# NoemieJaquier/GaBOtorch

Measured on AMD Instinct MI355X. Metric: SPD affine-invariant kernel-matrix build, pairs/sec (N=4096,d=10), higher is better.
Workload: dtype f64

## Files before the change

gabotorch_amd/_lib.py:

```python
import ctypes
import os

_PKG = os.path.dirname(os.path.abspath(__file__))
LIB_PATH = os.environ.get("GABO_HIP_LIB", os.path.join(_PKG, "libgabo_hip.so"))

GABO_OK = 0
GABO_ERR_DIM, GABO_ERR_ARG, GABO_ERR_NOT_SPD, GABO_ERR_LAUNCH = -1, -2, -3, -4
GABO_OUT_GAUSSIAN, GABO_OUT_DISTANCE, GABO_OUT_LAPLACE, GABO_SYMMETRIC = 0, 1, 2, 4
GABO_OUT_ZONAL = 3
GABO_SPD_REG_MAX_DIM = 12
GABO_SPD_BWD_REG_MAX_DIM = 16
GABO_SPD_FWD_REG_MAX_DIM = 20
GABO_SPD_MAX_DIM = 32
GABO_TR_NESTED_MAX_DIM = 24
(GABO_SPD_EXP, GABO_SPD_LOG, GABO_SPD_INNER, GABO_SPD_NORM, GABO_SPD_DIST, GABO_SPD_EGRAD2RGRAD, GABO_SPD_EHESS2RHESS,
 GABO_SPD_LOGM, GABO_SPD_EXPM, GABO_SPD_SQRTM, GABO_SPD_EIGMAX, GABO_SPD_EIGMIN) = range(12)
GABO_ACQ_EXPECTED_IMPROVEMENT, GABO_ACQ_POSTERIOR_MEAN = 0, 1
GABO_GP_MLL_MAX_N = 160
GABO_GP_FACTOR_MAX_N = 96
GABO_GP_MLL_LARGE_MAX_N = 2048
GABO_GRAM_EIG_MAX_N = 1024
GABO_GRAM_EIG_LDS_MAX_N = 192
GABO_GP_POSTERIOR_MAX_M = 1048576
GABO_MVN_SAMPLE_MAX_M = 192
# ... 15 lines not shown

_c = ctypes
_P, _I64, _I, _D, _SZ = _c.c_void_p, _c.c_int64, _c.c_int, _c.c_double, _c.c_size_t

class AcqParams(_c.Structure):
    _fields_ = [("train_factors", _c.c_void_p), ("alpha", _c.c_void_p), ("linv", _c.c_void_p), ("linv_t", _c.c_void_p),
                ("n", _c.c_int64), ("beta", _c.c_double), ("flags", _c.c_int), ("mean", _c.c_double), ("outputscale", _c.c_double),
                ("kxx", _c.c_double), ("best_f", _c.c_double), ("kind", _c.c_int), ("maximize", _c.c_int), ("out_sign", _c.c_double)]


class SweepConfig(_c.Structure):
    _fields_ = [("acq", AcqParams), ("d", _c.c_int), ("min_eig", _c.c_double), ("max_eig", _c.c_double), ("n_constraints", _c.c_int),
                ("constraint_kind", _c.c_int * 8), ("constraint_bound", _c.c_double * 8), ("strict", _c.c_int),
                ("delta_bar", _c.c_double), ("delta0", _c.c_double), ("delta_cons", _c.c_double), ("theta", _c.c_double), ("kappa", _c.c_double),
                ("mininner", _c.c_int), ("maxinner", _c.c_int), ("rho_prime", _c.c_double), ("rho_regularization", _c.c_double),
                ("mingradnorm", _c.c_double), ("maxiter", _c.c_int64)]


class SphereAcqParams(_c.Structure):
    _fields_ = [("train", _c.c_void_p), ("train_t", _c.c_void_p), ("alpha", _c.c_void_p), ("linv", _c.c_void_p), ("linv_t", _c.c_void_p),
                ("n", _c.c_int64), ("dim", _c.c_int), ("beta", _c.c_double), ("flags", _c.c_int), ("mean", _c.c_double),
                ("outputscale", _c.c_double), ("kxx", _c.c_double), ("best_f", _c.c_double), ("kind", _c.c_int), ("maximize", _c.c_int),
                ("out_sign", _c.c_double), ("series", _c.c_void_p), ("series_levels", _c.c_int), ("series_dim", _c.c_int)]


class SphereSweepConfig(_c.Structure):
    _fields_ = [("acq", SphereAcqParams), ("delta_bar", _c.c_double), ("delta0", _c.c_double), ("theta", _c.c_double), ("kappa", _c.c_double),
                ("mininner", _c.c_int), ("maxinner", _c.c_int), ("exact_hessian", _c.c_int), ("rho_prime", _c.c_double),
                ("rho_regularization", _c.c_double), ("mingradnorm", _c.c_double), ("maxiter", _c.c_int64)]


class SphereSweepConstraints(_c.Structure):
    _fields_ = [("n_constraints", _c.c_int), ("n_equalities", _c.c_int), ("kind", _c.c_int * 8), ("index", _c.c_int * 8), ("bound", _c.c_double * 8),
                ("centres", _c.c_void_p), ("n_centres", _c.c_int), ("strict", _c.c_int), ("delta_cons", _c.c_double)]


class ReconSolveOptions(_c.Structure):
    _fields_ = [(k, _c.c_double) for k in ("bound", "rho_init", "thetarho", "tau", "starting_tolgradnorm", "ending_tolgradnorm", "gammas_fact",
                                          "minstepsize", "maxtime")] + [("maxiter", _c.c_int64)] + \
               [(k, _c.c_double) for k in ("cg_minstepsize", "cg_maxtime", "cg_orth_value")] + [("cg_maxiter", _c.c_int64), ("lookahead", _c.c_int64), ("host_threads", _c.c_int64)]


class ReconSolveLog(_c.Structure):
    _fields_ = [(k, _c.c_int64) for k in ("outer_iterations", "inner_iterations", "evaluations", "launches")] + [("stop_reason", _c.c_int)] + \
               [(k, _c.c_double) for k in ("violation", "rho", "gamma", "final_cost", "seconds", "seconds_evaluator")] + [("host_threads", _c.c_int64)]


ReconEvalFn = _c.CFUNCTYPE(_c.c_int, _c.c_void_p, _c.c_int64, *([_c.POINTER(_c.c_double)] * 7))

SIGNATURES = {
    "gabo_version": (_I, []),
    "gabo_spd_ai_workspace_bytes": (_SZ, [_I64, _I64, _I64, _I]),
    "gabo_spd_ai_pairwise": (_I, [_P, _P, _P, _P, _I64, _I64, _I64, _I, _I64, _I64, _D, _I, _P, _SZ, _P, _P]),
    "gabo_spd_ai_backward": (_I, [_P, _P, _P, _P, _I64, _I64, _I64, _I, _I64, _I64, _I64, _I64, _I64, _D, _I, _P, _SZ, _P, _P]),
    "gabo_spd_ai_backward2_workspace_bytes": (_SZ, [_I64, _I64, _I64, _I]),
    "gabo_spd_ai_backward2": (_I, [_P, _P, _P, _P, _P, _P, _P, _I64, _I64, _I64, _I, _I64, _I64, _I64, _I64, _I64, _D, _I, _P, _SZ, _P, _P]),
    "gabo_nested_spd_gram_workspace_bytes": (_SZ, [_I64, _I64, _I64, _I]),
    "gabo_nested_spd_gram": (_I, [_P, _P, _P, _P, _I64, _I64, _I64, _I, _I, _I, _D, _I, _P, _SZ, _P, _P]),
    "gabo_nested_spd_matern_gram": (_I, [_P, _P, _P, _P, _I64, _I64, _I64, _I, _I, _D, _I, _P, _SZ, _P, _P]),
    "gabo_sphere_pairwise": (_I, [_P, _P, _P, _I64, _I64, _I64, _I, _I64, _I64, _D, _I, _I, _P]),
    "gabo_sphere_ktable_doubles": (_I64, []),
    "gabo_sphere_pairwise_uses_ktable": (_I, [_I64, _I64, _I64, _I, _D, _I, _I]),
    "gabo_sphere_ktable_build": (_I, [_D, _P, _P]),
    "gabo_sphere_pairwise_cached": (_I, [_P, _P, _P, _I64, _I64, _I64, _I, _I64, _I64, _D, _I, _I, _P, _P]),
    "gabo_sphere_from_inner": (_I, [_P, _P, _I64, _D, _I, _I, _P]),
    "gabo_sphere_zonal_from_inner": (_I, [_P, _P, _I64, _P, _I, _I, _P]),
    "gabo_sphere_zonal_pairwise": (_I, [_P, _P, _P, _I64, _I64, _I64, _I, _I64, _I64, _P, _I, _I, _I, _I, _P]),
    "gabo_spd_manifold_op": (_I, [_I, _P, _P, _P, _P, _P, _P, _I64, _I, _P, _P]),
    "gabo_spd_project": (_I, [_P, _P, _P, _I64, _I, _I, _P]),
    "gabo_spd_logm_mandel": (_I, [_P, _P, _I64, _I, _P]),
    "gabo_frobenius_pairwise": (_I, [_P, _P, _P, _I64, _I64, _I64, _I, _I64, _I64, _D, _I, _P]),
    "gabo_gp_acquisition": (_I, [_P, _P, _P, _P, _P, _P, _I64, _I64, _D, _D, _D, _D, _I, _I, _D, _P]),
    "gabo_gp_mll": (_I, [_P, _P, _I64, _D, _D, _D, _D, _P, _P]),
    "gabo_gp_mll_gram": (_I, [_P, _P, _I64, _D, _D, _D, _P, _P, _P]),
    "gabo_gp_mll_series": (_I, [_P, _P, _I64, _P, _P, _I, _I, _D, _D, _D, _P, _P]),
    "gabo_gp_factor": (_I, [_P, _P, _I64, _D, _D, _D, _P, _P, _P, _P, _P, _P]),
    "gabo_gp_mll_large_workspace_bytes": (_SZ, [_I64]),
    "gabo_gp_mll_large": (_I, [_P, _P, _I64, _D, _D, _D, _D, _I, _P, _P, _P, _SZ, _P]),
    "gabo_flat_matern_pairwise": (_I, [_P, _P, _P, _I64, _I64, _I64, _I, _I64, _I64, _D, _I, _P]),
    "gabo_flat_matern_backward": (_I, [_P, _P, _P, _P, _I64, _I64, _I64, _I, _I64, _I64, _I64, _I64, _I64, _D, _I, _D, _P]),
    "gabo_flat_matern_from_distance": (_I, [_P, _P, _I64, _D, _I, _I, _P]),
    "gabo_gp_mll_matern": (_I, [_P, _P, _I64, _D, _I, _D, _D, _D, _P, _P]),
    "gabo_spd_ai_logdiag": (_I, [_P, _P, _P, _I64, _I64, _I, _P]),
    "gabo_spd_ai_spectral_features": (_I, [_P, _P, _P, _P, _P, _I64, _I64, _I, _P]),
    "gabo_gram_extreme_eig_workspace_bytes": (_SZ, [_I64, _I64, _I64]),
    "gabo_gram_extreme_eig": (_I, [_P, _I64, _I64, _P, _I64, _P, _P, _SZ, _P]),
    "gabo_gp_posterior_joint_workspace_bytes": (_SZ, [_I64, _I64]),
    "gabo_gp_posterior_joint": (_I, [_P, _P, _P, _P, _I64, _I64, _D, _D, _P, _P, _P, _SZ, _P]),
    "gabo_mvn_sample": (_I, [_P, _P, _I64, _I64, _c.c_uint64, _P, _P, _P, _P, _P]),
    "gabo_mvn_base_samples": (_I, [_P, _I64, _I64, _c.c_uint64, _P]),
    "gabo_gp_condition_workspace_bytes": (_SZ, [_I64, _I64]),
    "gabo_gp_condition": (_I, [_P, _P, _P, _I64, _P, _P, _P, _I64, _D, _D, _D, _P, _P, _P, _P, _P, _P, _SZ, _P, _P]),
    "gabo_spd_acq_max_train": (_I64, [_I]),
    "gabo_spd_acq_prepare_train": (_I, [_P, _P, _I64, _I, _P, _P]),
    "gabo_spd_acq_eval": (_I, [_P, _P, _P, _P, _P, _P, _P, _P, _I64, _I64, _I, _D, _I, _D, _D, _D, _D, _I, _I, _D, _P, _P, _P]),
    "gabo_spd_tcg_workspace_bytes": (_SZ, [_I64, _I, _I]),
    "gabo_spd_tcg_running_offset": (_SZ, [_I64, _I, _I]),
    "gabo_spd_tcg_begin": (_I, [_P, _P, _P, _P, _P, _P, _P, _SZ, _I64, _I, _I, _P, _P]),
    "gabo_spd_tcg_begin_rand": (_I, [_P, _P, _P, _I64, _I, _I, _P]),
    "gabo_spd_tcg_fd_point": (_I, [_P, _P, _I64, _I, _I, _P]),
    "gabo_spd_tcg_step": (_I, [_P, _P, _P, _I64, _I, _I, _I, _D, _D, _D, _I, _P]),
    "gabo_spd_tcg_end": (_I, [_P, _P, _P, _P, _I64, _I, _I, _P]),
    "gabo_spd_sample": (_I, [_P, _I64, _I, _D, _D, _c.c_uint64, _I, _P]),
    "gabo_spd_sample_range": (_I, [_P, _I64, _I64, _I, _D, _D, _c.c_uint64, _I, _P]),
    "gabo_nested_sphere_epilogue": (_I, [_P, _P, _I64, _I, _D, _I, _P]),
    "gabo_nested_sphere_epilogue_backward": (_I, [_P, _P, _P, _I64, _I, _D, _P]),
# ... 95 lines not shown
```

gabotorch_amd/csrc/riemannian_mean.hip:

```cpp
#include "gabo_device.hpp"
#include "spd_prep.hpp"
#include "spd_eigvec.hpp"
#include "../../include/gabo_hip.h"

#define GABO_MEAN_MAX_DIM 10
#define GABO_MEAN_TWO_WAVE_MAX_DIM 8
#define GABO_MEAN_TWO_PASS_MIN_DIM 4
#define GABO_SPHERE_MEAN_MAX_DIM 512

namespace gabo {

struct MeanPlan {
    int64_t chunks, cpb, P;
};

static int device_cu_count() {
    int dev = 0, v = 0;
    if (hipGetDevice(&dev) == hipSuccess && hipDeviceGetAttribute(&v, hipDeviceAttributeMultiprocessorCount, dev) == hipSuccess && v > 0) return v;
    return 256;
}

static MeanPlan mean_plan(int64_t batch, int64_t n, int waves_per_simd) {
    MeanPlan pl;
    pl.chunks = (n + 63) / 64;
    const int64_t slots = (int64_t)4 * device_cu_count() * waves_per_simd;
    int64_t want = slots / batch;
    if (want < 1) want = 1;
    pl.P = pl.chunks < want ? pl.chunks : want;
    pl.cpb = (pl.chunks + pl.P - 1) / pl.P;
    pl.P = (pl.chunks + pl.cpb - 1) / pl.cpb;
    return pl;
}

__device__ __forceinline__ double weight_scale(const double* __restrict__ weights, int64_t b, int64_t n, int lane) {
    if (!weights) return 1.0 / (double)n;
    double a = 0.0;
    for (int64_t j = lane; j < n; j += 64) a += weights[b * n + j];
    return 1.0 / wave_allsum(a);
}

template <int D>
__global__ __launch_bounds__(64, (D > GABO_MEAN_TWO_WAVE_MAX_DIM ? 1 : 2)) void spd_mean_accumulate_kernel(
    const double* __restrict__ Winv, const double* __restrict__ G, const double* __restrict__ weights, const double* __restrict__ scale,
    double* __restrict__ partial, int64_t n, int P, int64_t cpb, int64_t pstride) {
    constexpr int T = tri_size(D);
    __shared__ double acc[T * 64];
    const int lane = threadIdx.x;
    const int64_t b = blockIdx.x / P;
    const int64_t p = blockIdx.x - b * P;
    const double* W = Winv + b * T;
    const double* Gb = G + b * T * n;
    const double sc = scale[b];
    static_for<T>([&](auto ee) { acc[decltype(ee)::value * 64 + lane] = 0.0; });
    const int64_t jbegin = p * cpb * 64;
    const int64_t jend = (jbegin + cpb * 64 < n) ? jbegin + cpb * 64 : n;
    for (int64_t j0 = jbegin; j0 < jend; j0 += 64) {
        const int64_t j = j0 + lane;
        const bool live = j < n;
        const int64_t jc = live ? j : n - 1;
        const double* Gj = Gb + jc;
        double m[T];
        static_for<T>([&](auto ee) { m[decltype(ee)::value] = 0.0; });
        static_for<D>([&](auto cc) {
            constexpr int col = decltype(cc)::value;
            double g[D - col], c[D - col];
            static_for<D - col>([&](auto kk) { g[decltype(kk)::value] = Gj[(int64_t)tri(col + decltype(kk)::value, col) * n]; });
            static_for<D - col>([&](auto rr) {
                constexpr int r = col + decltype(rr)::value;
                double a = W[tri(r, col)] * g[0];
                static_for<r - col>([&](auto kk) {
                    constexpr int k = col + 1 + decltype(kk)::value;
                    a = __builtin_fma(W[tri(r, k)], g[k - col], a);
                });
// ... 300 lines not shown
```

gabotorch_amd/csrc/spd_pairwise.hip:

```cpp
#include "spd_pairwise_body.hpp"


namespace gabo {
int launch_spd_ai_prepared(int d, double* out, int64_t batch, int64_t n1, int64_t n2, bool shared1, bool shared2, double beta, int flags,
                           double* ws, hipStream_t st) {
    const int64_t s1 = shared1 ? 0 : 1, s2 = shared2 ? 0 : 1;
    switch (d) {
        case 2: return launch_spd_ai<2>(nullptr, nullptr, out, nullptr, batch, n1, n2, s1, s2, beta, flags, ws, nullptr, st, true);
        case 3: return launch_spd_ai<3>(nullptr, nullptr, out, nullptr, batch, n1, n2, s1, s2, beta, flags, ws, nullptr, st, true);
        case 4: return launch_spd_ai<4>(nullptr, nullptr, out, nullptr, batch, n1, n2, s1, s2, beta, flags, ws, nullptr, st, true);
    }
    return GABO_ERR_DIM;
}
}

extern "C" {

size_t gabo_spd_ai_workspace_bytes(int64_t batch, int64_t n1, int64_t n2, int d) {
    if (batch < 0 || n1 < 0 || n2 < 0 || d < 1) return 0;
    const size_t packed = (size_t)(batch * (n1 + n2)) * (size_t)gabo::tri_size(d) * sizeof(double);
    const size_t generic = (size_t)(2 * batch * n1) * (size_t)d * (size_t)d * sizeof(double);
    if (d > GABO_SPD_FWD_REG_MAX_DIM) return generic;
    if (d > GABO_SPD_REG_MAX_DIM) return packed > generic ? packed : generic;
    return packed;
}

int gabo_spd_ai_pairwise(const double* x1, const double* x2, double* out, double* dist_out, int64_t batch, int64_t n1, int64_t n2, int d,
                         int64_t x1_batch_stride, int64_t x2_batch_stride, double beta, int flags, void* workspace,
                         size_t workspace_bytes, int* status, gabo_stream_t stream) {
    if (batch < 0 || n1 < 0 || n2 < 0 || x1_batch_stride < 0 || x2_batch_stride < 0) return GABO_ERR_ARG;
    if (d < 2 || d > GABO_SPD_MAX_DIM) return GABO_ERR_DIM;
    if (batch == 0 || n1 == 0 || n2 == 0) return GABO_OK;
    if (!x1 || !x2 || !out || !workspace || !status) return GABO_ERR_ARG;
    if (workspace_bytes < gabo_spd_ai_workspace_bytes(batch, n1, n2, d)) return GABO_ERR_ARG;
    if ((flags & GABO_SYMMETRIC) && (n1 != n2 || batch > 65535)) return GABO_ERR_ARG;
    hipStream_t st = (hipStream_t)stream;
    double* ws = (double*)workspace;
    if (d > GABO_SPD_FWD_REG_MAX_DIM)
        return gabo::launch_spd_ai_generic(x1, x2, out, dist_out, batch, n1, n2, d, x1_batch_stride, x2_batch_stride, beta, flags, ws,
                                           status, st);
#define GABO_CASE(DD) \
    case DD:          \
        return gabo::launch_spd_ai<DD>(x1, x2, out, dist_out, batch, n1, n2, x1_batch_stride, x2_batch_stride, beta, flags, ws, status, st);
    switch (d) {
#ifdef GABO_ONLY_DIM
        GABO_CASE(GABO_ONLY_DIM)
#else
        GABO_CASE(2) GABO_CASE(3) GABO_CASE(4) GABO_CASE(5) GABO_CASE(6) GABO_CASE(7) GABO_CASE(8) GABO_CASE(9) GABO_CASE(10)
        GABO_CASE(11) GABO_CASE(12)
#endif
    }
#undef GABO_CASE
#ifndef GABO_ONLY_DIM
    if (d > GABO_SPD_REG_MAX_DIM)
        return gabo::launch_spd_ai_wide(d, x1, x2, out, dist_out, batch, n1, n2, x1_batch_stride, x2_batch_stride, beta, flags, ws, status, st);
#endif
    return GABO_ERR_DIM;
}

}
```

gabotorch_amd/csrc/spd_pairwise_body.hpp:

```cpp
#pragma once
#include "gabo_device.hpp"
#include "spd_eig.hpp"
#include "spd_prep.hpp"
#include "gabo_mirror.hpp"
#include "spd_generic.hpp"
#include "gabo_log_tab.hpp"
#include "gabo_exp_tab256.hpp"
#include "gabo_acosh2_table.hpp"
#include "../../include/gabo_hip.h"

#ifndef GABO_PAIR_WAVES
#define GABO_PAIR_WAVES 2
#else
#define GABO_PAIR_WAVES_FORCED 1
#endif

namespace gabo {

typedef const double __attribute__((address_space(1)))* spd_gcol_ptr;

struct SpdGcolBuffer {
    __amdgpu_buffer_rsrc_t rsrc;
    int voff;
    int stride_bytes;
    __device__ __forceinline__ double operator[](int k) const {
        return __builtin_bit_cast(double, __builtin_amdgcn_raw_buffer_load_b64(rsrc, voff, k * stride_bytes, 0));
    }
};
struct SpdGcolPointer {
    spd_gcol_ptr p;
    int64_t stride;
    __device__ __forceinline__ double operator[](int k) const { return p[(int64_t)k * stride]; }
};

template <int D, int WLIM>
struct SpdWGroups {
    int n = 0;
    int col[tri_size(D)] = {}, r0[tri_size(D)] = {}, r1[tri_size(D)] = {};
    constexpr SpdWGroups() {
        static_assert(WLIM >= D, "a row of the first column must fit a group");
        for (int c = D - 1; c >= 0; --c) {
            for (int r = c; r < D;) {
                int sum = 0;
                col[n] = c, r0[n] = r;
                while (r < D && sum + (r - c + 1) <= WLIM) sum += r - c + 1, ++r;
                r1[n++] = r;
            }
        }
    }
};
#ifndef GABO_PAIR_WLIM
#define GABO_PAIR_WLIM 16
#endif
template <int D, int AHEAD, class GCOL>
__device__ __forceinline__ void ai_congruence_staged(const double* __restrict__ W, const GCOL& Gj, double (&m)[tri_size(D)]) {
    constexpr SpdWGroups<D, (GABO_PAIR_WLIM < D ? D : GABO_PAIR_WLIM)> kG{};
    double gq[D][D];
    double wq[2][D][D];
    double c[D];
    auto issue_g = [&](auto ss) {
        constexpr int col = D - 1 - decltype(ss)::value;
// ... 93 lines not shown

struct Spd2Col {
    double g00, g10, g11, lg;
};
__device__ __forceinline__ double ai_sumsq2(const double* __restrict__ W, const Spd2Col& g, double lw, const LogTabRegs& lr,
                                            const double* __restrict__ ltab, double tiny) {
    const double c00 = W[0] * g.g00, c11 = W[2] * g.g11;
    const double c10 = __builtin_fma(W[1], g.g00, W[2] * g.g10);
    const double m00 = c00 * c00, m10d = (c10 + c10) * c00, m11 = __builtin_fma(c10, c10, c11 * c11);
    const double tr = m00 + m11, df = m00 - m11;
    const double root = sqrt_nz(__builtin_fma(df, df, __builtin_fma(m10d, m10d, tiny)));
    const double l1 = log_tab(0.5 * (tr + root), lr, ltab);
    const double l2 = __builtin_fma(2.0, lw + g.lg, -l1);
    return __builtin_fma(l1, l1, l2 * l2);
}

__device__ __forceinline__ double finish(double dist, double beta, int mode) {
    if (mode == GABO_OUT_DISTANCE) return dist;
    if (mode == GABO_OUT_LAPLACE) return exp(-(dist * beta));
    return exp(-((dist * dist) * beta));
}

#ifndef GABO_PAIR_TWO_WAVE_MAX_DIM
#define GABO_PAIR_TWO_WAVE_MAX_DIM 14
#endif
#ifndef GABO_QL_EPS2_GAUSS
#define GABO_QL_EPS2_GAUSS 1e-14
#endif
constexpr bool spd_pair_gauss_only_instantiated(int d) { return d > 2 && d != 12; }
#ifndef GABO_PAIR_ORIENT
constexpr int spd_pair_gauss_only_orientation(int d) { return d == 14 ? kQlOrientCol0 : kQlOrientLast; }
#else
constexpr int spd_pair_gauss_only_orientation(int d) { return GABO_PAIR_ORIENT; }
#endif
#ifndef GABO_PAIR_SWEEPCTL
constexpr int spd_pair_gauss_only_sweepctl(int d) { return d == 20 ? kQlCtlPlain : (kQlCtlDenormalZero | kQlCtlHwSqrt | kQlCtlStageThreshold); }
#else
constexpr int spd_pair_gauss_only_sweepctl(int d) { return GABO_PAIR_SWEEPCTL; }
#endif
#ifndef GABO_PAIR_WAVES_FORCED
constexpr int spd_pair_gauss_only_waves(int d) { return d > GABO_PAIR_TWO_WAVE_MAX_DIM ? 1 : (d == 10 ? 3 : GABO_PAIR_WAVES); }
#else
constexpr int spd_pair_gauss_only_waves(int d) { return d > GABO_PAIR_TWO_WAVE_MAX_DIM ? 1 : GABO_PAIR_WAVES; }
#endif
#ifndef GABO_PAIR_AHEAD
constexpr int spd_pair_gauss_only_ahead(int d) { return d == 10 && spd_pair_gauss_only_waves(d) == 3 ? 2 : 0; }
#else
constexpr int spd_pair_gauss_only_ahead(int d) { return d == 10 ? GABO_PAIR_AHEAD : 0; }
#endif
template <int D, bool GAUSS_ONLY, bool BUFFER_ONLY>
__global__ __launch_bounds__(256, (GAUSS_ONLY ? spd_pair_gauss_only_waves(D) : (D > GABO_PAIR_TWO_WAVE_MAX_DIM ? 1 : GABO_PAIR_WAVES))) void spd_ai_pairwise_kernel(const double* __restrict__ Winv, const double* __restrict__ G,
                                                              double* __restrict__ out, double* __restrict__ dist_out_arg,
                                                              int64_t n1, int64_t n2,
                                                              int64_t w_batch_stride, int64_t g_batch_stride, int rows,
                                                              int col_blocks, int row_chunks, int64_t sym_tiles, double beta, int flags) {
    constexpr int T = tri_size(D);
    static_assert(GAUSS_ONLY == BUFFER_ONLY && (spd_pair_gauss_only_instantiated(D) || !GAUSS_ONLY), "instantiations that launch_spd_ai selects");
    const int mode = GAUSS_ONLY ? GABO_OUT_GAUSSIAN : (flags & GABO_OUT_MASK);
    double* const dist_out = GAUSS_ONLY ? nullptr : dist_out_arg;
    constexpr bool kTabExp = D <= 4;
    __shared__ double tab[kTabExp ? 64 : 1];
    __shared__ __attribute__((aligned(16))) double ltab[512];
    for (int k = threadIdx.x; k < 512; k += blockDim.x) ltab[k] = kLogTab[k];
    double ec[6], ec3 = 0.0;
    if constexpr (kTabExp) {
        if (threadIdx.x < 64) tab[threadIdx.x] = kExp2Tab[threadIdx.x];
    }
    __syncthreads();
    if constexpr (kTabExp) {
        static_for<6>([&](auto k) { ec[decltype(k)::value] = kExpTabC[decltype(k)::value]; });
        ec3 = ec[3];
        asm volatile("" : "+v"(ec3));
    }
    int64_t cg, rc, b;
    if (flags & GABO_SYMMETRIC) {
        const int64_t per_batch = sym_tiles;
        b = blockIdx.x / per_batch;
        int64_t t = blockIdx.x - b * per_batch;
        cg = 0;
        for (;;) {
            int64_t cnt = ((cg + 1) * (int64_t)blockDim.x + rows - 1) / rows;
            if (cnt > row_chunks) cnt = row_chunks;
            if (t < cnt) break;
            t -= cnt;
            ++cg;
        }
        rc = t;
    } else {
        const int64_t bid = blockIdx.x;
        cg = bid % col_blocks;
        rc = (bid / col_blocks) % row_chunks;
        b = bid / ((int64_t)col_blocks * row_chunks);
    }
    const int64_t j0 = cg * blockDim.x;
    const int64_t j = j0 + threadIdx.x;
    const int64_t jc = j < n2 ? j : n2 - 1;
    const int64_t i0 = rc * rows;
    const int64_t i1 = (i0 + rows < n1) ? i0 + rows : n1;
    if ((flags & GABO_SYMMETRIC) && j0 + (int64_t)(threadIdx.x | 63) < i0) return;
    const double* Gj = G + b * g_batch_stride + jc;
    double* ob = out + b * n1 * n2;
    const int64_t jw = j0 + (threadIdx.x & ~63);
    const bool use_buffer = BUFFER_ONLY || (D > 2 && (int64_t)T * n2 * 8 < (1ll << 31));
    SpdGcolBuffer gbuf;
    {
        const double* gw = G + b * g_batch_stride + (jw < n2 ? jw : n2 - 1);
        uint64_t a = (uint64_t)gw;
        a = ((uint64_t)(uint32_t)__builtin_amdgcn_readfirstlane((int)(a >> 32)) << 32) | (uint32_t)__builtin_amdgcn_readfirstlane((int)a);
        gbuf.rsrc = __builtin_amdgcn_make_buffer_rsrc((void*)a, 0, 0x7fffffff, 0x00020000);
        gbuf.voff = (int)((jc - (jw < n2 ? jw : n2 - 1)) * 8);
        gbuf.stride_bytes = (int)(n2 * 8);
    }
    Spd2Col col2;
    double lw_lane = 0.0, tiny = 1e-290;
    LogTabRegs lr2;
    if constexpr (D == 2) {
        lr2 = LogTabRegs::load();
        asm volatile("" : "+s"(tiny));
        col2.g00 = Gj[0];
        col2.g10 = Gj[n2];
        col2.g11 = Gj[2 * n2];
        col2.lg = log_tab(col2.g00 * col2.g11, lr2, ltab);
        int64_t ir = i0 + (threadIdx.x & 63);
        ir = ir < n1 ? ir : n1 - 1;
        const double* Wr = Winv + b * w_batch_stride + ir * T;
        lw_lane = log_tab(Wr[0] * Wr[2], lr2, ltab);
    }
    double eps2 = (mode == GABO_OUT_GAUSSIAN && !dist_out) ? GABO_QL_EPS2_GAUSS : 0.0;
    asm volatile("" : "+s"(eps2));
    if constexpr (GAUSS_ONLY && BUFFER_ONLY) {
        const int nrows = __builtin_amdgcn_readfirstlane((int)(i1 - i0));
        const int64_t jrel = j - i0;
        const int rmax = j >= n2 ? -1 : ((flags & GABO_SYMMETRIC) ? (jrel < 0 ? -1 : (jrel > rows - 1 ? rows - 1 : (int)jrel)) : rows - 1);
        const double* W = Winv + b * w_batch_stride + i0 * T;
        char* orow = reinterpret_cast<char*>(ob + i0 * n2 + j);
        for (int r = 0; r < nrows; ++r, W += T) {
            SpdGcolBuffer gb = gbuf;
            asm volatile("" : "+v"(gb.voff));
            asm volatile("" : "+s"(gb.stride_bytes));
            const double s = ai_sumsq<D, spd_pair_gauss_only_orientation(D), spd_pair_gauss_only_sweepctl(D), spd_pair_gauss_only_ahead(D)>(W, gb, ltab, eps2);
            double val;
            if constexpr (kTabExp) {
                val = exp_neg_tab(-((s + 1e-15) * beta), ec, ec3, tab);
                val = s != s ? s : val;
            } else {
                val = exp(-((s + 1e-15) * beta));
            }
            if (r <= rmax) *reinterpret_cast<double*>(orow) = val;
            orow += (unsigned)gb.stride_bytes;
        }
// ... 124 lines not shown
    const double q00 = g00 * sg, q10 = g10 * sg, q11 = g11 * sg;
    double* orow = out + b * n1 * n2 + i0 * n2 + j;
    const int nrows = __builtin_amdgcn_readfirstlane((int)(i1 - i0));
    const int64_t jrel = j - i0;
    const int rmax = j >= n2 ? -1 : (SYM ? (jrel < 0 ? -1 : (jrel > GABO_GAUSS2_MAX_ROWS - 1 ? GABO_GAUSS2_MAX_ROWS - 1 : (int)jrel)) : GABO_GAUSS2_MAX_ROWS - 1);
    typedef double g2_v2d __attribute__((ext_vector_type(2)));
    if (!SYM && j >= n2) return;
    for (int r = 0; r < nrows; ++r, orow += n2) {
        const g2_v2d wa = *reinterpret_cast<const g2_v2d*>(wrow + 4 * r);
        const g2_v2d wb = *reinterpret_cast<const g2_v2d*>(wrow + 4 * r + 2);
        const double w0 = wa[0], w1 = wa[1], w2 = wb[0], arow = wb[1];
        const double hh = __builtin_fma(w0, q00, -(w2 * q11));
        const double cc = __builtin_fma(w1, q00, w2 * q10);
        const double tau = __builtin_fma(cc, cc, __builtin_fma(hh, hh, 1.0));
        const unsigned hi = (unsigned)__double2hiint(tau);
        static_assert(kAcosh2MBits == 4 && kAcosh2Slots == 256, "row index = 8 bits");
        const unsigned off = __umul24((hi >> 16) & 0xffu, (unsigned)(kAcosh2Stride * sizeof(double)));
        const double t = tau - __hiloint2double((int)(hi & ~((1u << (20 - kAcosh2MBits)) - 1u)), 0);
        const g2_v2d* row = reinterpret_cast<const g2_v2d*>(reinterpret_cast<const char*>(atab) + off);
        static_assert(kAcosh2Deg == 7, "four coefficient pairs");
        const g2_v2d c67 = row[3], c45 = row[2], c23 = row[1], c01 = row[0];
        double ya = __builtin_fma(c67[1], t, c67[0]);
        ya = __builtin_fma(ya, t, c45[1]);
        ya = __builtin_fma(ya, t, c45[0]);
        ya = __builtin_fma(ya, t, c23[1]);
        ya = __builtin_fma(ya, t, c23[0]);
        ya = __builtin_fma(ya, t, c01[1]);
        ya = __builtin_fma(ya, t, c01[0]);
        if (__builtin_expect(__any(!(tau < ec[5])), 0)) {
            if (!(tau < ec[5])) {
                const double dl = log(tau + __builtin_sqrt(__builtin_fma(tau, tau, -1.0)));
                ya = -(sscale * sscale) * __builtin_fma(dl, dl, 0.5e-15);
            }
        }
        const double sp = arow + bcol;
        const double y = __builtin_fma(-sp, sp, ya);
        const double km = y + ec[4];
        const double kk = km - ec[4];
        const double rr = y - kk;
        double p = __builtin_fma(rr, c4v, ec[2]);
        p = __builtin_fma(p, rr, ec[1]);
        p = __builtin_fma(p, rr, ec[0]);
        p = p * rr;
        const int ki = __double2loint(km);
        const double e = etab[ki & 255];
        const double val = __builtin_ldexp(__builtin_fma(e, p, e), ki >> 8);
        if (!SYM || r <= rmax) {
            if constexpr (NT) __builtin_nontemporal_store(val, orow);
            else *orow = val;
        }
    }
}

template <int D>
static int launch_spd_ai(const double* x1, const double* x2, double* out, double* dist_out, int64_t batch, int64_t n1, int64_t n2,
                         int64_t s1, int64_t s2, double beta, int flags, double* ws, int* status, hipStream_t st, bool prepared = false) {
    constexpr int T = tri_size(D);
    const int64_t b1 = (s1 == 0) ? 1 : batch;
    const int64_t b2 = (s2 == 0) ? 1 : batch;
    double* W = ws;
    double* G = ws + b1 * n1 * T;
    if (!prepared) launch_spd_prep<D>(x1, x2, W, G, b1, b2, n1, n2, s1, s2, status, st, 1);
#ifndef GABO_PAIR_THREADS
#define GABO_PAIR_THREADS (D >= 7 ? 64 : 256)
#endif
    int threads = n2 >= 256 ? GABO_PAIR_THREADS : (n2 > 128 ? 192 : (n2 > 64 ? 128 : 64));
    int64_t col_blocks = (n2 + threads - 1) / threads;
#ifndef GABO_PAIR_ROWS_D2
#define GABO_PAIR_ROWS_D2 16
#endif
#ifndef GABO_PAIR_ROWS
#define GABO_PAIR_ROWS (D >= 9 ? 8 : 16)
#endif
#ifndef GABO_PAIR_ROWS_GAUSS2
#define GABO_PAIR_ROWS_GAUSS2 64
#endif
    const bool gauss2 = D == 2 && (flags & GABO_OUT_MASK) == GABO_OUT_GAUSSIAN && !dist_out && beta >= 0.0;
    int rows = D == 2 ? (gauss2 ? GABO_PAIR_ROWS_GAUSS2 : GABO_PAIR_ROWS_D2) : GABO_PAIR_ROWS;
    while (rows > 1 && col_blocks * ((n1 + rows - 1) / rows) * batch < (rows > 16 ? 1024 : 4096)) rows >>= 1;
    int64_t row_chunks = (n1 + rows - 1) / rows;
    int64_t sym_tiles = 0;
    if (flags & GABO_SYMMETRIC) {
        for (int64_t cg = 0; cg < col_blocks; ++cg) {
            int64_t cnt = ((cg + 1) * threads + rows - 1) / rows;
            sym_tiles += cnt < row_chunks ? cnt : row_chunks;
        }
    }
    int64_t nblocks = ((flags & GABO_SYMMETRIC) ? sym_tiles : col_blocks * row_chunks) * batch;
    if (nblocks > 0x7fffffffLL) return GABO_ERR_ARG;
    bool special2 = false;
    if constexpr (D == 2) special2 = gauss2 && rows <= GABO_GAUSS2_MAX_ROWS;
    if (special2) {
        const bool streaming = batch * n1 * n2 * 8 > (32ll << 20) && !(flags & GABO_SYMMETRIC);
#define GABO_GAUSS2_LAUNCH(...)                                                                                                     \
        hipLaunchKernelGGL((spd_ai_gauss2_kernel<__VA_ARGS__>), dim3((unsigned)nblocks), dim3(threads), 0, st, W, G, out, n1, n2,           \
                           (s1 == 0) ? (int64_t)0 : n1 * T, (s2 == 0) ? (int64_t)0 : n2 * T, rows, (int)col_blocks, (int)row_chunks,       \
                           sym_tiles, beta, flags)
        if (flags & GABO_SYMMETRIC) GABO_GAUSS2_LAUNCH(false, true);
        else if (streaming) GABO_GAUSS2_LAUNCH(true, false);
        else GABO_GAUSS2_LAUNCH(false, false);
#undef GABO_GAUSS2_LAUNCH
    } else {
#define GABO_PAIR_LAUNCH(...)                                                                                                             \
        hipLaunchKernelGGL((spd_ai_pairwise_kernel<D, __VA_ARGS__>), dim3((unsigned)nblocks), dim3(threads), 0, st, W, G, out, dist_out, n1, n2, \
                           (s1 == 0) ? (int64_t)0 : n1 * T, (s2 == 0) ? (int64_t)0 : n2 * T, rows, (int)col_blocks, (int)row_chunks,       \
                           sym_tiles, beta, flags)
        bool gauss_only = false;
        if constexpr (spd_pair_gauss_only_instantiated(D)) {
            gauss_only = (flags & GABO_OUT_MASK) == GABO_OUT_GAUSSIAN && !dist_out && (int64_t)T * n2 * 8 < (1ll << 31);
            if (gauss_only) GABO_PAIR_LAUNCH(true, true);
        }
        if (!gauss_only) GABO_PAIR_LAUNCH(false, false);
#undef GABO_PAIR_LAUNCH
    }
    if (flags & GABO_SYMMETRIC) {
        int tiles = (int)((n1 + 31) / 32);
        hipLaunchKernelGGL((mirror_upper_kernel<0>), dim3((unsigned)((int64_t)tiles * (tiles + 1) / 2), (unsigned)batch), dim3(256), 0, st,
                           out, n1, tiles);
        if (dist_out)
            hipLaunchKernelGGL((mirror_upper_kernel<0>), dim3((unsigned)((int64_t)tiles * (tiles + 1) / 2), (unsigned)batch), dim3(256), 0,
                               st, dist_out, n1, tiles);
    }
    return hipGetLastError() == hipSuccess ? GABO_OK : GABO_ERR_LAUNCH;
}

}

namespace gabo {
int launch_spd_ai_prepared(int d, double* out, int64_t batch, int64_t n1, int64_t n2, bool shared1, bool shared2, double beta, int flags,
                           double* ws, hipStream_t st);
int launch_spd_ai_wide2(int d, const double* x1, const double* x2, double* out, double* dist_out, int64_t batch, int64_t n1, int64_t n2,
                        int64_t s1, int64_t s2, double beta, int flags, double* ws, int* status, hipStream_t st);
int launch_spd_ai_wide3(int d, const double* x1, const double* x2, double* out, double* dist_out, int64_t batch, int64_t n1, int64_t n2,
                        int64_t s1, int64_t s2, double beta, int flags, double* ws, int* status, hipStream_t st);
int launch_spd_ai_wide(int d, const double* x1, const double* x2, double* out, double* dist_out, int64_t batch, int64_t n1, int64_t n2,
                       int64_t s1, int64_t s2, double beta, int flags, double* ws, int* status, hipStream_t st);
}
```

include/gabo_hip.h:

```cpp
#ifndef GABO_HIP_H
#define GABO_HIP_H

#include <stddef.h>
#include <stdint.h>

#ifdef __cplusplus
extern "C" {
#endif

typedef void* gabo_stream_t;

#define GABO_OK 0
#define GABO_ERR_DIM (-1)
#define GABO_ERR_ARG (-2)
#define GABO_ERR_NOT_SPD (-3)
#define GABO_ERR_LAUNCH (-4)

#define GABO_OUT_GAUSSIAN 0
#define GABO_OUT_DISTANCE 1
#define GABO_OUT_LAPLACE 2
#define GABO_OUT_ZONAL 3
#define GABO_OUT_MASK 3
#define GABO_SYMMETRIC 4
#define GABO_METRIC_AFFINE_INVARIANT 0
#define GABO_METRIC_LOG_EUCLIDEAN 8
#define GABO_METRIC_FROBENIUS 16
#define GABO_METRIC_MASK 24

#define GABO_SPD_REG_MAX_DIM 12
#define GABO_SPD_BWD_REG_MAX_DIM 16
#define GABO_SPD_FWD_REG_MAX_DIM 20
#define GABO_SPD_MAX_DIM 32

int gabo_version(void);

size_t gabo_spd_ai_workspace_bytes(int64_t batch, int64_t n1, int64_t n2, int d);
int gabo_spd_ai_pairwise(const double* x1, const double* x2, double* out, double* dist_out, int64_t batch, int64_t n1,
                         int64_t n2, int d, int64_t x1_batch_stride, int64_t x2_batch_stride, double beta, int flags,
                         void* workspace, size_t workspace_bytes, int* status, gabo_stream_t stream);

int gabo_spd_ai_backward(const double* x1, const double* x2, const double* grad_out, double* grad_x1, int64_t batch, int64_t n1,
                         int64_t n2, int d, int64_t x1_batch_stride, int64_t x2_batch_stride, int64_t go_batch_stride,
                         int64_t go_row_stride, int64_t go_col_stride, double beta, int flags, void* workspace,
                         size_t workspace_bytes, int* status, gabo_stream_t stream);

size_t gabo_spd_ai_backward2_workspace_bytes(int64_t batch, int64_t n1, int64_t n2, int d);
int gabo_spd_ai_backward2(const double* x1, const double* x2, const double* grad_out, const double* u, double* hv_x1, double* d_grad_out,
                          double* mixed_x2, int64_t batch, int64_t n1, int64_t n2, int d, int64_t x1_batch_stride, int64_t x2_batch_stride,
                          int64_t go_batch_stride, int64_t go_row_stride, int64_t go_col_stride, double beta, int flags, void* workspace,
                          size_t workspace_bytes, int* status, gabo_stream_t stream);

int gabo_sphere_pairwise(const double* x1, const double* x2, double* out, int64_t batch, int64_t n1, int64_t n2,
                         int dim, int64_t x1_batch_stride, int64_t x2_batch_stride, double beta, int flags, int diag,
                         gabo_stream_t stream);
int64_t gabo_sphere_ktable_doubles(void);
int gabo_sphere_pairwise_uses_ktable(int64_t batch, int64_t n1, int64_t n2, int dim, double beta, int flags, int diag);
int gabo_sphere_ktable_build(double beta, double* table, gabo_stream_t stream);
int gabo_sphere_pairwise_cached(const double* x1, const double* x2, double* out, int64_t batch, int64_t n1, int64_t n2,
                                int dim, int64_t x1_batch_stride, int64_t x2_batch_stride, double beta, int flags, int diag,
                                const double* ktable, gabo_stream_t stream);

int gabo_sphere_from_inner(const double* inner, double* out, int64_t n, double beta, int flags, int order, gabo_stream_t stream);

int gabo_sphere_zonal_from_inner(const double* inner, double* out, int64_t n, const double* coeff_host, int n_coeff, int series_dim,
                                 gabo_stream_t stream);
int gabo_sphere_zonal_pairwise(const double* x1, const double* x2, double* out, int64_t batch, int64_t n1, int64_t n2, int dim,
                               int64_t x1_batch_stride, int64_t x2_batch_stride, const double* coeff_host, int n_coeff, int series_dim,
                               int flags, int diag, gabo_stream_t stream);

int gabo_mandel_to_matrix(const double* vec, double* mat, int64_t n, int d, gabo_stream_t stream);
int gabo_matrix_to_mandel(const double* mat, double* vec, int64_t n, int d, gabo_stream_t stream);

#define GABO_SPD_EXP 0
#define GABO_SPD_LOG 1
#define GABO_SPD_INNER 2
#define GABO_SPD_NORM 3
#define GABO_SPD_DIST 4
#define GABO_SPD_EGRAD2RGRAD 5
#define GABO_SPD_EHESS2RHESS 6
#define GABO_SPD_LOGM 7
#define GABO_SPD_EXPM 8
#define GABO_SPD_SQRTM 9
#define GABO_SPD_EIGMAX 10
#define GABO_SPD_EIGMIN 11
int gabo_spd_manifold_op(int op, const double* a, const double* b, const double* c, const double* e, double* out, double* out2,
                         int64_t n, int d, int* status, gabo_stream_t stream);

int gabo_spd_project(const double* x_mandel, const double* w, double* y_mandel, int64_t n, int D, int dl, gabo_stream_t stream);

int gabo_spd_logm_mandel(const double* x_mandel, double* y_mandel, int64_t n, int d, gabo_stream_t stream);

int gabo_frobenius_pairwise(const double* x1, const double* x2, double* out, int64_t batch, int64_t n1, int64_t n2, int d,
// ... 375 lines not shown
```

Baseline: 7.976 billion.

## Shrink row-chunk sizes near the end of the grid to balance the final wave

Replaces the uniform rows-per-block split of the SPD affine-invariant pairwise kernel with a multi-phase row schedule. The bulk of the rows keeps the default chunk size, and the tail of the last batch is split into progressively smaller power-of-two chunks, sized from an estimate of how many wave slots the device has. The aim is to shorten the partially filled last wave of blocks. The CU count query is now cached per device, and an API entry exposes the computed schedule. In exchange, block-index decoding in the kernel becomes more complex, and the small tail chunks reuse x1 rows less.

```diff
diff --git a/gabotorch_amd/_lib.py b/gabotorch_amd/_lib.py
--- a/gabotorch_amd/_lib.py
+++ b/gabotorch_amd/_lib.py
@@ -91,6 +91,7 @@
     "gabo_version": (_I, []),
     "gabo_spd_ai_workspace_bytes": (_SZ, [_I64, _I64, _I64, _I]),
     "gabo_spd_ai_pairwise": (_I, [_P, _P, _P, _P, _I64, _I64, _I64, _I, _I64, _I64, _D, _I, _P, _SZ, _P, _P]),
+    "gabo_spd_ai_row_schedule": (_I, [_I64, _I64, _I64, _I, _I, _I64, _P, _I]),
     "gabo_spd_ai_backward": (_I, [_P, _P, _P, _P, _I64, _I64, _I64, _I, _I64, _I64, _I64, _I64, _I64, _D, _I, _P, _SZ, _P, _P]),
     "gabo_spd_ai_backward2_workspace_bytes": (_SZ, [_I64, _I64, _I64, _I]),
     "gabo_spd_ai_backward2": (_I, [_P, _P, _P, _P, _P, _P, _P, _I64, _I64, _I64, _I, _I64, _I64, _I64, _I64, _I64, _D, _I, _P, _SZ, _P, _P]),
diff --git a/gabotorch_amd/csrc/gabo_device_info.hpp b/gabotorch_amd/csrc/gabo_device_info.hpp
--- /dev/null
+++ b/gabotorch_amd/csrc/gabo_device_info.hpp
@@ -0,0 +1,19 @@
+#pragma once
+#include <atomic>
+#include <hip/hip_runtime.h>
+
+namespace gabo {
+
+inline int device_cu_count() {
+    constexpr int kMaxDevices = 64;
+    static std::atomic<int> cached[kMaxDevices];
+    int dev = 0, v = 0;
+    if (hipGetDevice(&dev) != hipSuccess) return 256;
+    const bool slot = dev >= 0 && dev < kMaxDevices;
+    if (slot && (v = cached[dev].load(std::memory_order_relaxed)) > 0) return v;
+    if (hipDeviceGetAttribute(&v, hipDeviceAttributeMultiprocessorCount, dev) != hipSuccess || v <= 0) return 256;
+    if (slot) cached[dev].store(v, std::memory_order_relaxed);
+    return v;
+}
+
+}
diff --git a/gabotorch_amd/csrc/riemannian_mean.hip b/gabotorch_amd/csrc/riemannian_mean.hip
--- a/gabotorch_amd/csrc/riemannian_mean.hip
+++ b/gabotorch_amd/csrc/riemannian_mean.hip
@@ -1,4 +1,5 @@
 #include "gabo_device.hpp"
+#include "gabo_device_info.hpp"
 #include "spd_prep.hpp"
 #include "spd_eigvec.hpp"
 #include "../../include/gabo_hip.h"
@@ -13,12 +14,6 @@
 struct MeanPlan {
     int64_t chunks, cpb, P;
 };
-
-static int device_cu_count() {
-    int dev = 0, v = 0;
-    if (hipGetDevice(&dev) == hipSuccess && hipDeviceGetAttribute(&v, hipDeviceAttributeMultiprocessorCount, dev) == hipSuccess && v > 0) return v;
-    return 256;
-}
 
 static MeanPlan mean_plan(int64_t batch, int64_t n, int waves_per_simd) {
     MeanPlan pl;
diff --git a/gabotorch_amd/csrc/spd_pairwise.hip b/gabotorch_amd/csrc/spd_pairwise.hip
--- a/gabotorch_amd/csrc/spd_pairwise.hip
+++ b/gabotorch_amd/csrc/spd_pairwise.hip
@@ -23,6 +23,21 @@
     if (d > GABO_SPD_FWD_REG_MAX_DIM) return generic;
     if (d > GABO_SPD_REG_MAX_DIM) return packed > generic ? packed : generic;
     return packed;
+}
+
+int gabo_spd_ai_row_schedule(int64_t batch, int64_t n1, int64_t n2, int d, int flags, int64_t slots, int64_t* out, int cap) {
+    if (batch < 1 || n1 < 1 || n2 < 1 || slots < 0 || cap < 0 || (cap > 0 && !out)) return GABO_ERR_ARG;
+    if (d < 2 || d > GABO_SPD_FWD_REG_MAX_DIM) return GABO_ERR_DIM;
+    if ((flags & GABO_SYMMETRIC) && (n1 != n2 || batch > 65535)) return GABO_ERR_ARG;
+    const gabo::SpdAiPlan plan = gabo::spd_ai_plan(d, batch, n1, n2, 1.0, flags, false, slots);
+    if (plan.sched.n == 0 || plan.nblocks > 0x7fffffffLL) return GABO_ERR_ARG;
+    const gabo::SpdRowSchedule& s = plan.sched;
+    for (int q = 0; q < s.n && q < cap; ++q) {
+        out[3 * q] = s.first_row[q];
+        out[3 * q + 1] = (int64_t)1 << s.lg[q];
+        out[3 * q + 2] = (q + 1 < s.n ? s.first_chunk[q + 1] : s.total_chunks) - s.first_chunk[q];
+    }
+    return s.n;
 }
 
 int gabo_spd_ai_pairwise(const double* x1, const double* x2, double* out, double* dist_out, int64_t batch, int64_t n1, int64_t n2, int d,
diff --git a/gabotorch_amd/csrc/spd_pairwise_body.hpp b/gabotorch_amd/csrc/spd_pairwise_body.hpp
--- a/gabotorch_amd/csrc/spd_pairwise_body.hpp
+++ b/gabotorch_amd/csrc/spd_pairwise_body.hpp
@@ -7,6 +7,8 @@
 #include "gabo_log_tab.hpp"
 #include "gabo_exp_tab256.hpp"
 #include "gabo_acosh2_table.hpp"
+#include "gabo_device_info.hpp"
+#include "spd_row_schedule.hpp"
 #include "../../include/gabo_hip.h"
 
 #ifndef GABO_PAIR_WAVES
@@ -206,9 +208,29 @@
 __global__ __launch_bounds__(256, (GAUSS_ONLY ? spd_pair_gauss_only_waves(D) : (D > GABO_PAIR_TWO_WAVE_MAX_DIM ? 1 : GABO_PAIR_WAVES))) void spd_ai_pairwise_kernel(const double* __restrict__ Winv, const double* __restrict__ G,
                                                               double* __restrict__ out, double* __restrict__ dist_out_arg,
                                                               int64_t n1, int64_t n2,
-                                                              int64_t w_batch_stride, int64_t g_batch_stride, int rows,
-                                                              int col_blocks, int row_chunks, int64_t sym_tiles, double beta, int flags) {
+                                                              int64_t w_batch_stride, int64_t g_batch_stride, SpdRowSchedule sched,
+                                                              int64_t sym_tiles, double beta, int flags) {
     constexpr int T = tri_size(D);
+    int64_t cg = 0, b = 0, i0 = 0;
+    int rows = 1 << sched.lg[0];
+    if (!(flags & GABO_SYMMETRIC)) {
+        const unsigned t = blockIdx.x / (unsigned)sched.col_blocks, bb = t / (unsigned)sched.total_chunks;
+        const int y = (int)(t - bb * (unsigned)sched.total_chunks);
+        cg = blockIdx.x - t * (unsigned)sched.col_blocks;
+        b = bb;
+        int fc = 0, lg = sched.lg[0];
+        int64_t fr = 0;
+        if (b == sched.last_batch) {
+            static_for<kSpdRowPhases - 1>([&](auto qq) {
+                constexpr int q = 1 + decltype(qq)::value;
+                if (y >= sched.first_chunk[q]) fc = sched.first_chunk[q], lg = sched.lg[q], fr = sched.first_row[q];
+            });
+        } else if (y >= sched.bulk_chunks) {
+            return;
+        }
+        rows = 1 << lg;
+        i0 = fr + ((int64_t)(y - fc) << lg);
+    }
     static_assert(GAUSS_ONLY == BUFFER_ONLY && (spd_pair_gauss_only_instantiated(D) || !GAUSS_ONLY), "instantiations that launch_spd_ai selects");
     const int mode = GAUSS_ONLY ? GABO_OUT_GAUSSIAN : (flags & GABO_OUT_MASK);
     double* const dist_out = GAUSS_ONLY ? nullptr : dist_out_arg;
@@ -226,9 +248,8 @@
         ec3 = ec[3];
         asm volatile("" : "+v"(ec3));
     }
-    int64_t cg, rc, b;
     if (flags & GABO_SYMMETRIC) {
-        const int64_t per_batch = sym_tiles;
+        const int64_t per_batch = sym_tiles, row_chunks = sched.total_chunks;
         b = blockIdx.x / per_batch;
         int64_t t = blockIdx.x - b * per_batch;
         cg = 0;
@@ -239,17 +260,11 @@
             t -= cnt;
             ++cg;
         }
-        rc = t;
-    } else {
-        const int64_t bid = blockIdx.x;
-        cg = bid % col_blocks;
-        rc = (bid / col_blocks) % row_chunks;
-        b = bid / ((int64_t)col_blocks * row_chunks);
+        i0 = t * rows;
     }
     const int64_t j0 = cg * blockDim.x;
     const int64_t j = j0 + threadIdx.x;
     const int64_t jc = j < n2 ? j : n2 - 1;
-    const int64_t i0 = rc * rows;
     const int64_t i1 = (i0 + rows < n1) ? i0 + rows : n1;
     if ((flags & GABO_SYMMETRIC) && j0 + (int64_t)(threadIdx.x | 63) < i0) return;
     const double* Gj = G + b * g_batch_stride + jc;
@@ -480,6 +495,59 @@
     }
 }
 
+#ifndef GABO_PAIR_THREADS
+#define GABO_PAIR_THREADS (D >= 7 ? 64 : 256)
+#endif
+#ifndef GABO_PAIR_ROWS_D2
+#define GABO_PAIR_ROWS_D2 16
+#endif
+#ifndef GABO_PAIR_ROWS
+#define GABO_PAIR_ROWS (D >= 9 ? 8 : 16)
+#endif
+#ifndef GABO_PAIR_SCHED_K
+#define GABO_PAIR_SCHED_K 2
+#endif
+#ifndef GABO_PAIR_ROWS_GAUSS2
+#define GABO_PAIR_ROWS_GAUSS2 64
+#endif
+
+struct SpdAiPlan {
+    int threads, rows;
+    int64_t col_blocks, sym_tiles, nblocks;
+    bool special2, gauss_only;
+    SpdRowSchedule sched;
+};
+static inline SpdAiPlan spd_ai_plan(const int D, int64_t batch, int64_t n1, int64_t n2, double beta, int flags, bool has_dist, int64_t slots) {
+    SpdAiPlan p = {};
+    const int64_t T = tri_size(D);
+    const bool sym = (flags & GABO_SYMMETRIC) != 0, gaussian = (flags & GABO_OUT_MASK) == GABO_OUT_GAUSSIAN && !has_dist;
+    p.threads = n2 >= 256 ? GABO_PAIR_THREADS : (n2 > 128 ? 192 : (n2 > 64 ? 128 : 64));
+    p.col_blocks = (n2 + p.threads - 1) / p.threads;
+    const bool gauss2 = D == 2 && gaussian && beta >= 0.0;
+    int rows = D == 2 ? (gauss2 ? GABO_PAIR_ROWS_GAUSS2 : GABO_PAIR_ROWS_D2) : GABO_PAIR_ROWS;
+    while (rows > 1 && p.col_blocks * ((n1 + rows - 1) / rows) * batch < (rows > 16 ? 1024 : 4096)) rows >>= 1;
+    p.rows = rows;
+    p.special2 = gauss2 && rows <= GABO_GAUSS2_MAX_ROWS;
+    p.gauss_only = !p.special2 && spd_pair_gauss_only_instantiated(D) && gaussian && T * n2 * 8 < (1ll << 31);
+    if (sym || p.special2 || GABO_PAIR_SCHED_K == 0) {
+        p.sched = spd_row_single_phase(n1, rows);
+    } else {
+        const int waves = p.gauss_only ? spd_pair_gauss_only_waves(D) : (D > GABO_PAIR_TWO_WAVE_MAX_DIM ? 1 : GABO_PAIR_WAVES);
+        if (slots <= 0) slots = (int64_t)4 * device_cu_count() * waves;
+        p.sched = spd_row_schedule(n1, p.col_blocks * (p.threads / 64), rows, slots, GABO_PAIR_SCHED_K);
+    }
+    p.sched.last_batch = (int)(batch - 1);
+    if (sym) {
+        for (int64_t cg = 0; cg < p.col_blocks; ++cg) {
+            int64_t cnt = ((cg + 1) * p.threads + rows - 1) / rows;
+            p.sym_tiles += cnt < p.sched.total_chunks ? cnt : p.sched.total_chunks;
+        }
+    }
+    p.nblocks = (sym ? p.sym_tiles : p.col_blocks * p.sched.total_chunks) * batch;
+    p.sched.col_blocks = (int)(p.col_blocks <= 0x7fffffff ? p.col_blocks : 0x7fffffff);
+    return p;
+}
+
 template <int D>
 static int launch_spd_ai(const double* x1, const double* x2, double* out, double* dist_out, int64_t batch, int64_t n1, int64_t n2,
                          int64_t s1, int64_t s2, double beta, int flags, double* ws, int* status, hipStream_t st, bool prepared = false) {
@@ -488,57 +556,31 @@
     const int64_t b2 = (s2 == 0) ? 1 : batch;
     double* W = ws;
     double* G = ws + b1 * n1 * T;
+    const SpdAiPlan plan = spd_ai_plan(D, batch, n1, n2, beta, flags, dist_out != nullptr, 0);
+    if (plan.sched.n == 0 || plan.nblocks > 0x7fffffffLL || batch > 0x7fffffffLL) return GABO_ERR_ARG;
     if (!prepared) launch_spd_prep<D>(x1, x2, W, G, b1, b2, n1, n2, s1, s2, status, st, 1);
-#ifndef GABO_PAIR_THREADS
-#define GABO_PAIR_THREADS (D >= 7 ? 64 : 256)
-#endif
-    int threads = n2 >= 256 ? GABO_PAIR_THREADS : (n2 > 128 ? 192 : (n2 > 64 ? 128 : 64));
-    int64_t col_blocks = (n2 + threads - 1) / threads;
-#ifndef GABO_PAIR_ROWS_D2
-#define GABO_PAIR_ROWS_D2 16
-#endif
-#ifndef GABO_PAIR_ROWS
-#define GABO_PAIR_ROWS (D >= 9 ? 8 : 16)
-#endif
-#ifndef GABO_PAIR_ROWS_GAUSS2
-#define GABO_PAIR_ROWS_GAUSS2 64
-#endif
-    const bool gauss2 = D == 2 && (flags & GABO_OUT_MASK) == GABO_OUT_GAUSSIAN && !dist_out && beta >= 0.0;
-    int rows = D == 2 ? (gauss2 ? GABO_PAIR_ROWS_GAUSS2 : GABO_PAIR_ROWS_D2) : GABO_PAIR_ROWS;
-    while (rows > 1 && col_blocks * ((n1 + rows - 1) / rows) * batch < (rows > 16 ? 1024 : 4096)) rows >>= 1;
-    int64_t row_chunks = (n1 + rows - 1) / rows;
-    int64_t sym_tiles = 0;
-    if (flags & GABO_SYMMETRIC) {
-        for (int64_t cg = 0; cg < col_blocks; ++cg) {
-            int64_t cnt = ((cg + 1) * threads + rows - 1) / rows;
-            sym_tiles += cnt < row_chunks ? cnt : row_chunks;
-        }
-    }
-    int64_t nblocks = ((flags & GABO_SYMMETRIC) ? sym_tiles : col_blocks * row_chunks) * batch;
-    if (nblocks > 0x7fffffffLL) return GABO_ERR_ARG;
-    bool special2 = false;
-    if constexpr (D == 2) special2 = gauss2 && rows <= GABO_GAUSS2_MAX_ROWS;
-    if (special2) {
-        const bool streaming = batch * n1 * n2 * 8 > (32ll << 20) && !(flags & GABO_SYMMETRIC);
+    const int threads = plan.threads;
+    const int64_t nblocks = plan.nblocks, sym_tiles = plan.sym_tiles;
+    if (plan.special2) {
+        if constexpr (D == 2) {
+            const bool streaming = batch * n1 * n2 * 8 > (32ll << 20) && !(flags & GABO_SYMMETRIC);
 #define GABO_GAUSS2_LAUNCH(...)                                                                                                     \
-        hipLaunchKernelGGL((spd_ai_gauss2_kernel<__VA_ARGS__>), dim3((unsigned)nblocks), dim3(threads), 0, st, W, G, out, n1, n2,           \
-                           (s1 == 0) ? (int64_t)0 : n1 * T, (s2 == 0) ? (int64_t)0 : n2 * T, rows, (int)col_blocks, (int)row_chunks,       \
-                           sym_tiles, beta, flags)
-        if (flags & GABO_SYMMETRIC) GABO_GAUSS2_LAUNCH(false, true);
-        else if (streaming) GABO_GAUSS2_LAUNCH(true, false);
-        else GABO_GAUSS2_LAUNCH(false, false);
+            hipLaunchKernelGGL((spd_ai_gauss2_kernel<__VA_ARGS__>), dim3((unsigned)nblocks), dim3(threads), 0, st, W, G, out, n1, n2,       \
+                               (s1 == 0) ? (int64_t)0 : n1 * T, (s2 == 0) ? (int64_t)0 : n2 * T, plan.rows, (int)plan.col_blocks,          \
+                               plan.sched.total_chunks, sym_tiles, beta, flags)
+            if (flags & GABO_SYMMETRIC) GABO_GAUSS2_LAUNCH(false, true);
+            else if (streaming) GABO_GAUSS2_LAUNCH(true, false);
+            else GABO_GAUSS2_LAUNCH(false, false);
 #undef GABO_GAUSS2_LAUNCH
+        }
     } else {
 #define GABO_PAIR_LAUNCH(...)                                                                                                             \
         hipLaunchKernelGGL((spd_ai_pairwise_kernel<D, __VA_ARGS__>), dim3((unsigned)nblocks), dim3(threads), 0, st, W, G, out, dist_out, n1, n2, \
-                           (s1 == 0) ? (int64_t)0 : n1 * T, (s2 == 0) ? (int64_t)0 : n2 * T, rows, (int)col_blocks, (int)row_chunks,       \
-                           sym_tiles, beta, flags)
-        bool gauss_only = false;
+                           (s1 == 0) ? (int64_t)0 : n1 * T, (s2 == 0) ? (int64_t)0 : n2 * T, plan.sched, sym_tiles, beta, flags)
         if constexpr (spd_pair_gauss_only_instantiated(D)) {
-            gauss_only = (flags & GABO_OUT_MASK) == GABO_OUT_GAUSSIAN && !dist_out && (int64_t)T * n2 * 8 < (1ll << 31);
-            if (gauss_only) GABO_PAIR_LAUNCH(true, true);
-        }
-        if (!gauss_only) GABO_PAIR_LAUNCH(false, false);
+            if (plan.gauss_only) GABO_PAIR_LAUNCH(true, true);
+        }
+        if (!plan.gauss_only) GABO_PAIR_LAUNCH(false, false);
 #undef GABO_PAIR_LAUNCH
     }
     if (flags & GABO_SYMMETRIC) {
diff --git a/gabotorch_amd/csrc/spd_row_schedule.hpp b/gabotorch_amd/csrc/spd_row_schedule.hpp
--- /dev/null
+++ b/gabotorch_amd/csrc/spd_row_schedule.hpp
@@ -0,0 +1,65 @@
+#pragma once
+#include <cstdint>
+
+namespace gabo {
+
+constexpr int kSpdRowPhases = 6;
+
+struct SpdRowSchedule {
+    int n;
+    int col_blocks;
+    int last_batch;
+    int lg[kSpdRowPhases];
+    int first_chunk[kSpdRowPhases];
+    int total_chunks;
+    int64_t first_row[kSpdRowPhases];
+    int bulk_chunks;
+};
+
+inline SpdRowSchedule spd_row_single_phase(int64_t n1, int rows) {
+    SpdRowSchedule s = {};
+    int lg = 0;
+    while ((2 << lg) <= rows) ++lg;
+    for (int q = 0; q < kSpdRowPhases; ++q) s.first_chunk[q] = 0x7fffffff;
+    const int64_t chunks = (n1 + rows - 1) / rows;
+    if (n1 <= 0 || chunks >= 0x7fffffff) return s;
+    s.n = 1, s.lg[0] = lg, s.first_chunk[0] = 0, s.total_chunks = (int)chunks, s.bulk_chunks = (int)chunks;
+    return s;
+}
+
+inline SpdRowSchedule spd_row_schedule(int64_t n1, int64_t col_waves, int bulk, int64_t slots, int k) {
+    SpdRowSchedule s = {};
+    for (int q = 0; q < kSpdRowPhases; ++q) s.first_chunk[q] = 0x7fffffff;
+    if (n1 <= 0) return s;
+    if (col_waves < 1) col_waves = 1;
+    int64_t row = 0, chunk = 0;
+    auto phase = [&](int h, int64_t chunks) {
+        int lg = 0;
+        while ((2 << lg) <= h) ++lg;
+        s.lg[s.n] = lg, s.first_row[s.n] = row, s.first_chunk[s.n] = (int)chunk;
+        ++s.n, row += chunks * h, chunk += chunks;
+    };
+    for (int h = bulk; h >= 2; h = (h == bulk && h > 32) ? 16 : h / 2) {
+        const int64_t rem = n1 - row, need = ((int64_t)h * k * slots + col_waves - 1) / col_waves;
+        if (rem < need) continue;
+        int64_t chunks = (rem - need) / h + 1;
+        if (chunks > rem / h) chunks = rem / h;
+        if (chunks > 0) phase(h, chunks);
+    }
+    if (row < n1) phase(1, n1 - row);
+    if (s.n > 1 && s.lg[s.n - 1] > 0) {
+        const int h = 1 << s.lg[s.n - 1];
+        if (chunk - s.first_chunk[s.n - 1] == 1) --s.n;
+        row -= h, --chunk;
+        phase(1, h);
+    }
+    if (chunk >= 0x7fffffff) {
+        s.n = 0;
+        return s;
+    }
+    s.total_chunks = (int)chunk;
+    s.bulk_chunks = (int)((n1 + (1 << s.lg[0]) - 1) >> s.lg[0]);
+    return s;
+}
+
+}
diff --git a/include/gabo_hip.h b/include/gabo_hip.h
--- a/include/gabo_hip.h
+++ b/include/gabo_hip.h
@@ -38,6 +38,7 @@
 int gabo_spd_ai_pairwise(const double* x1, const double* x2, double* out, double* dist_out, int64_t batch, int64_t n1,
                          int64_t n2, int d, int64_t x1_batch_stride, int64_t x2_batch_stride, double beta, int flags,
                          void* workspace, size_t workspace_bytes, int* status, gabo_stream_t stream);
+int gabo_spd_ai_row_schedule(int64_t batch, int64_t n1, int64_t n2, int d, int flags, int64_t slots, int64_t* out, int cap);
 
 int gabo_spd_ai_backward(const double* x1, const double* x2, const double* grad_out, double* grad_x1, int64_t batch, int64_t n1,
                          int64_t n2, int d, int64_t x1_batch_stride, int64_t x2_batch_stride, int64_t go_batch_stride,
```

After: 8.014 billion (median of 6 runs). No clear change (+0.5%).
